# robustrobotics/multi_view_stereonet

Measured on AMD Instinct MI355X. Metric: depthmaps/sec at 512x256, 64 hypotheses, 2 src views; L1 vs ref, higher is better.
Workload: dtype f32; 1 GPU; GTA-SfM-shaped 512x256, D=64 hypotheses, 2 source views, cost-volume filter + 5 refiners; global_batch=256, parallelism=dp1 (independent images, all-gather of metric rows)

## Files before the change

### include/mvsn_hip.h

```cpp
#ifndef MVSN_HIP_H
#define MVSN_HIP_H

#include <stddef.h>
#include <stdint.h>

#ifdef __cplusplus
extern "C" {
#endif

#define MVSN_ABI_VERSION 6

#define MVSN_E_BADARG (-1)
#define MVSN_E_TOOLARGE (-2)
#define MVSN_E_WORKSPACE (-3)

typedef void *mvsn_stream_t;

int mvsn_abi_version(void);
const char *mvsn_last_error(void);

int mvsn_plane_sweep_setup(const float *T_right_in_left, const float *K_lvl0, const float *K_lvl4,
                           int n_chains, int rows4, int cols4, int num_idepth_samples,
                           float *idepth_samples, float *H_lvl4, float *H_inc, float *H_lvl0_plane0,
                           float *baseline, mvsn_stream_t stream);
// ... 132 lines not shown
                         uint8_t *out, mvsn_stream_t stream);
int mvsn_fusion_gather(const float *maps, const int *view, const int *pixel, int n_views, long pixels_per_view,
                       long count, float *out, mvsn_stream_t stream);

int mvsn_channel_l2_norm(const float *x, int n, int channels, long pixels, float *out, mvsn_stream_t stream);
int mvsn_idepth_scale(const float *prior, const float *fx, int n, long pixels, float *out, mvsn_stream_t stream);
int mvsn_refiner_epilogue(const float *prior, const float *fx, const float *delta, int n, long pixels, float *out,
                          mvsn_stream_t stream);

int mvsn_upsample_bilinear(const float *in, int n, int channels, int rows_in, int cols_in, int rows_out,
                           int cols_out, float *out, mvsn_stream_t stream);
int mvsn_upsample_prior(const float *in, const float *fx, int n, int rows_in, int cols_in, int rows_out, int cols_out,
                        float *out, float *out_scaled, mvsn_stream_t stream);
int mvsn_upsample_mask(const uint8_t *in, int n, int channels, int rows_in, int cols_in, int rows_out,
                       int cols_out, uint8_t *out, mvsn_stream_t stream);

int mvsn_area_downsample(const float *in, int n, int channels, int rows_in, int cols_in, float *out,
                         mvsn_stream_t stream);

int mvsn_image_pyramid_supported(int rows, int cols, int levels);
int mvsn_image_pyramid(const float *in, int n, int channels, int rows, int cols, int levels, float *const *out_levels,
                       mvsn_stream_t stream);
int mvsn_prepare_cameras(const float *K, const float *T_right_in_left, int batch, int n_sources, int levels,
                         const int *level_sizes_dev, float *K_pyr, float *T_normalised, float *T_inverse_normalised,
                         float *baseline, mvsn_stream_t stream);

int mvsn_fuse_sources(const float *raw, const float *refined, const float *baseline, const uint8_t *mask,
                      int n_sources, int batch, int num_idepth_samples, int pixels, int refined_aliases_raw,
                      float *raw_out, float *refined_out, uint8_t *mask_out, mvsn_stream_t stream);

// ... 73 lines not shown
                       int64_t *result, void *workspace, size_t workspace_bytes, mvsn_stream_t stream);
int mvsn_tsdf_extract(const float *sdf_sum, const float *weight, const float *color_sum, int nx, int ny, int nz,
                      float voxel_size, float origin_x, float origin_y, float origin_z, float min_weight,
                      const void *workspace, size_t workspace_bytes, long n_vertices, long n_quads, float *vertices,
                      float *normals, uint8_t *colors, int64_t *faces, int64_t *cell, mvsn_stream_t stream);

int mvsn_copy(void *dst, const void *src, size_t nbytes, mvsn_stream_t stream);
int mvsn_copy_many(void *const *dst, const void *const *src, const size_t *nbytes, int count, mvsn_stream_t stream);
int mvsn_gather_focal(const float *const *K_pyr, int levels, int batch, float *fx, mvsn_stream_t stream);
int mvsn_gather_strided(const float *src, int count, long stride, float *dst, mvsn_stream_t stream);

int mvsn_debug_set_band_flags(int flags);

int mvsn_debug_set_wino_rowphase(int mode);

int mvsn_debug_wino_plan(const mvsn_conv_desc *desc, int carrying, int out[8]);

int mvsn_debug_conv_plan(const mvsn_conv_desc *desc, int mode, int out[8]);

int mvsn_selftest_mfma(mvsn_stream_t stream);

#ifdef __cplusplus
}
#endif
#endif
```

### multi_view_stereonet_amd/_native.py

```python
import ctypes
import os
from ctypes import c_char_p, c_int, c_long, c_size_t, c_void_p, POINTER, Structure

import torch

_LIB_PATH = os.path.join(os.path.dirname(os.path.abspath(__file__)), "libmvsn_hip.so")
_lib = None


class ConvDesc(Structure):
    _fields_ = [("n", c_int), ("c_in", c_int), ("c_out", c_int), ("depth", c_int), ("rows", c_int),
                ("cols", c_int), ("kd", c_int), ("kh", c_int), ("kw", c_int), ("stride", c_int),
                ("dilation", c_int), ("precision", c_int)]


class ApplyJob(Structure):
    _fields_ = [("x", c_void_p), ("stats", c_void_p), ("gamma", c_void_p), ("beta", c_void_p),
                ("residual", c_void_p), ("r_stats", c_void_p), ("r_gamma", c_void_p), ("r_beta", c_void_p),
                ("out", c_void_p), ("n", c_int), ("reverse", c_int), ("spatial", c_long)]


class TowerDesc(Structure):
    _fields_ = [("inp", c_void_p * 3), ("channels", c_int * 3), ("sample_mod", c_int * 3), ("block_scale", c_void_p),
                ("scale_mod", c_int), ("scale_block", c_int), ("head_chunks", c_int), ("n_blocks", c_int),
# ... 35 lines not shown
    "mvsn_conv_winograd_supported": (c_int, [POINTER(ConvDesc)]),
    "mvsn_conv_packed_floats": (c_size_t, [POINTER(ConvDesc)]),
    "mvsn_conv_pack_weights": (c_int, [POINTER(ConvDesc), c_void_p, c_void_p, c_void_p]),
    "mvsn_conv_num_tiles": (c_int, [POINTER(ConvDesc)]),
    "mvsn_conv_forward": (c_int, [POINTER(ConvDesc)] + [c_void_p] * 10 + [c_void_p]),
    "mvsn_conv_forward_blocks": (c_int, [POINTER(ConvDesc), c_void_p, POINTER(c_int), c_int] + [c_void_p] * 4 + [c_void_p]),
    "mvsn_conv_forward_carry": (c_int, [POINTER(ConvDesc)] + [c_void_p] * 8 + [POINTER(ApplyJob), POINTER(c_int), c_void_p]),
    "mvsn_groupnorm_finalize": (c_int, [c_void_p, c_int, c_int, c_void_p, c_void_p]),
    "mvsn_groupnorm_finalize_split_workspace_bytes": (c_size_t, [c_int, c_int]),
    "mvsn_groupnorm_finalize_split": (c_int, [c_void_p, c_int, c_int, c_void_p, c_void_p, c_size_t, c_void_p]),
    "mvsn_groupnorm_lrelu_apply": (c_int, [c_void_p] * 5 + [c_int, c_long, c_void_p, c_void_p]),
    "mvsn_groupnorm_lrelu_add2": (c_int, [c_void_p] * 8 + [c_int, c_long, c_void_p, c_void_p]),
    "mvsn_conv_to1_block": (c_int, [c_void_p] * 9 + [c_int] * 3 + [c_void_p, c_void_p]),
    "mvsn_debug_set_band_flags": (c_int, [c_int]),
    "mvsn_debug_set_wino_rowphase": (c_int, [c_int]),
    "mvsn_debug_wino_plan": (c_int, [POINTER(ConvDesc), c_int, POINTER(c_int * 8)]),
    "mvsn_debug_conv_plan": (c_int, [POINTER(ConvDesc), c_int, POINTER(c_int * 8)]),
    "mvsn_copy_many": (c_int, [c_void_p, c_void_p, c_void_p, c_int, c_void_p]),
    "mvsn_conv_to1_block_records": (c_int, [c_void_p] * 2 + [c_int] + [c_void_p] * 7 + [c_int] * 3 + [c_void_p, c_void_p]),
    "mvsn_groupnorm_lrelu_apply_records": (c_int, [c_void_p] * 2 + [c_int] + [c_void_p] * 6 + [c_int, c_long, c_void_p, c_void_p]),
    "mvsn_conv_to1_supported": (c_int, [c_int, c_int]),
    "mvsn_conv_to1_volume_norm": (c_int, [c_void_p] * 6 + [c_int] * 4 + [c_void_p, c_void_p]),
    "mvsn_conv_to1": (c_int, [c_void_p] * 5 + [c_int] * 5 + [c_void_p, c_void_p]),
    "mvsn_soft_argmin": (c_int, [c_void_p] * 2 + [c_int] * 3 + [c_void_p, c_void_p]),
    "mvsn_soft_argmin_confidence": (c_int, [c_void_p] * 2 + [c_int] * 3 + [c_void_p] * 2 + [c_void_p]),
    "mvsn_confidence_fuse_sources": (c_int, [c_void_p] + [c_int] * 3 + [c_void_p, c_void_p]),
    "mvsn_confidence_mask": (c_int, [c_void_p, c_void_p, c_long, ctypes.c_float, c_void_p, c_void_p]),
    "mvsn_fusion_gather": (c_int, [c_void_p] * 3 + [c_int, c_long, c_long, c_void_p, c_void_p]),
    "mvsn_channel_l2_norm": (c_int, [c_void_p, c_int, c_int, c_long, c_void_p, c_void_p]),
    "mvsn_idepth_scale": (c_int, [c_void_p, c_void_p, c_int, c_long, c_void_p, c_void_p]),
    "mvsn_refiner_epilogue": (c_int, [c_void_p, c_void_p, c_void_p, c_int, c_long, c_void_p, c_void_p]),
    "mvsn_upsample_bilinear": (c_int, [c_void_p] + [c_int] * 6 + [c_void_p, c_void_p]),
    "mvsn_upsample_prior": (c_int, [c_void_p, c_void_p] + [c_int] * 5 + [c_void_p] * 3),
    "mvsn_upsample_mask": (c_int, [c_void_p] + [c_int] * 6 + [c_void_p, c_void_p]),
    "mvsn_image_pyramid_supported": (c_int, [c_int] * 3),
    "mvsn_image_pyramid": (c_int, [c_void_p] + [c_int] * 5 + [POINTER(c_void_p), c_void_p]),
    "mvsn_prepare_cameras": (c_int, [c_void_p] * 2 + [c_int] * 3 + [c_void_p] * 5 + [c_void_p]),
    "mvsn_area_downsample": (c_int, [c_void_p] + [c_int] * 4 + [c_void_p, c_void_p]),
    "mvsn_fuse_sources": (c_int, [c_void_p] * 4 + [c_int] * 5 + [c_void_p] * 3 + [c_void_p]),
    "mvsn_idepth_reproject_blocks": (c_int, [c_int]),
    "mvsn_idepth_reproject": (c_int, [c_void_p] * 5 + [c_int] * 3 + [c_void_p] * 6 + [c_void_p]),
    "mvsn_occlusion_mask": (c_int, [c_void_p] * 4 + [c_int] * 2 + [c_void_p, c_void_p]),
    "mvsn_masked_l1": (c_int, [c_void_p] * 4 + [c_long, c_int, c_void_p, c_void_p]),
    "mvsn_tower_16x32": (c_int, [POINTER(TowerDesc), c_int, c_void_p]),
    "mvsn_depth_metrics_blocks": (c_int, [c_long]),
    "mvsn_depth_metrics": (c_int, [c_void_p] * 3 + [c_int, c_long, ctypes.c_float, ctypes.c_float, c_void_p, c_void_p, c_void_p]),
    "mvsn_fusion_workspace_bytes": (c_size_t, [c_int] * 4),
    "mvsn_fusion_consistency": (c_int, [c_void_p] * 6 + [c_int] * 5 + [ctypes.c_float] * 2 + [c_int] + [c_void_p] * 4 +
                                [c_size_t, c_void_p]),
# ... 132 lines not shown
```

### multi_view_stereonet_amd/csrc/mvsn_conv_wino.hip

```cpp
#include <type_traits>
#include <utility>

#include "mvsn_resident.h"
#include "mvsn_conv_wino.h"

namespace mvsn {

constexpr int WN_THREADS = 512, WN_WAVES = 8;
constexpr int WN_TY = 16, WN_TX = 32;
constexpr int WN_WIDE_TY = 10, WN_WIDE_TX = 40, WN_WIDE_PC = WN_WIDE_TX / 2, WN_WIDE_NP = (WN_WIDE_TY / 2) * WN_WIDE_PC;
constexpr int WN_ROLL_PR = 6, WN_ROLL_NP = WN_ROLL_PR * WN_WIDE_PC, WN_ROLL_HY = 2 * WN_ROLL_PR + 3;
constexpr int WN_TILE_RP = 3;
constexpr int wn_pa(int dil) { return (dil + 3) / 4 * 4; }
constexpr int WN_UFLOATS = 16 * 128;
constexpr int WN_MAX_CHUNKS = 9;
constexpr int WN_LDS_MAX = 160 * 1024;

__device__ floatx4 g_wn_zero16 = {0.f, 0.f, 0.f, 0.f};

#ifndef MVSN_WN_ABLATE
#define MVSN_WN_ABLATE 0
#endif

#ifndef MVSN_RD_ABLATE
// ... 167 lines not shown
  return WinoDiv{(unsigned)m, s};
}
__device__ __forceinline__ int wdiv(int n, WinoDiv f) { return (int)((__umulhi((unsigned)n, f.mul) + (unsigned)n) >> f.shift); }

struct WinoArgs {
  int n, cin, H, W, ntx, tiles, nchunks;
  WinoDiv fd_ntx;
  int cb0, cb1;
  const float *in1, *in2;
  size_t bs0, cs0;
  int rev;
  int D;
  int pr;
  WinoDiv fd_pr;
  int nty, rpy;
};

struct RideArgs {
  const float *x, *stats, *gamma, *beta;
  const float *res, *r_stats, *r_gamma, *r_beta;
  float *out;
  int units;
  WinoDiv fd_upp;
};
typedef const __attribute__((address_space(4))) float *wn_cfloat;
__device__ __forceinline__ float wn_sload(const float *p, size_t i) { return ((wn_cfloat)(size_t)p)[i]; }

__global__ void wino_pack_kernel(const float *__restrict__ w, int cin, int cout, int nchunks, int kd,
                                 float *__restrict__ out) {
  const int total = nchunks * WN_UFLOATS;
// ... 64 lines not shown
  const int nsteps = (g.nchunks + KS - 1) / KS;
  const int uchunks = VOL ? NSTAGE * KS : nsteps * KS;

  const int tid = threadIdx.x, lane = tid & 63;
  const int wave = __builtin_amdgcn_readfirstlane(tid >> 6);
  const size_t plane = (size_t)g.H * g.W;
  const int ptiles = ROLL ? g.tiles : (RP ? DIL * g.rpy * g.ntx : g.D * g.tiles);
  auto roll_item = [&](int t, int &zA, int &prA0, int &sA) {
    const int R0 = t * WN_ROLL_PR;
    zA = wdiv(R0, g.fd_pr);
    prA0 = R0 - zA * g.pr;
    sA = g.pr - prA0 < WN_ROLL_PR ? g.pr - prA0 : WN_ROLL_PR;
  };
  const int total = g.n * ptiles;
  const int G = gridDim.x;
  const int slot = xcd_tile_index(blockIdx.x, G);
#ifdef MVSN_WN_STAMPS
  unsigned long long *dbg = (blockIdx.x == gridDim.x / 3 && tid == 0) ? g_wn_stamps : nullptr;
  unsigned long long *dbg_lds = reinterpret_cast<unsigned long long *>(U + L.stamps(uchunks));
  int dbg_i = 0;
  bool dbg_on = true;
#endif
  WN_STAMP();

  if constexpr (!VOL) {
    const int runs = g.nchunks * (WN_UFLOATS / 256);
    for (int run = wave; run < runs; run += WN_WAVES)
      wn_dma16<ASM_DMA>(upk + (size_t)run * 256 + lane * 4, U + run * 256);
    if (uchunks != g.nchunks)
      *reinterpret_cast<floatx4 *>(U + g.nchunks * WN_UFLOATS + tid * 4) = floatx4{0.f, 0.f, 0.f, 0.f};
// ... 2 lines not shown
  float *bias_lds = U + L.bias(uchunks);
  if (tid < 32) bias_lds[tid] = bias ? bias[tid] : 0.0f;

  constexpr int STEP_PIECES = KS * 4 * PIECES;
  constexpr bool EVEN = STEP_PIECES % WN_WAVES == 0;
  constexpr int PER = EVEN ? STEP_PIECES / WN_WAVES : 2;
  static_assert(EVEN || (KS == 1 && PIECES == 3), "uneven DMA split only for the 12-piece case");
  static_assert(!EVEN || PIECES % PER == 0 || PER % PIECES == 0, "a wave's pieces stay within one channel");
  const int dch = EVEN ? (wave * PER) / PIECES : (wave & 3);
  const int dp0 = EVEN ? (wave * PER) % PIECES : (wave < 4 ? 0 : 2);
  const int dpn = EVEN ? (PER < PIECES ? PER : PIECES) : (wave < 4 ? 2 : 1);
  const float *zero = reinterpret_cast<const float *>(&g_wn_zero16);
  int pf_round = 0, pf_chunk = 0, pf_stage = 0;
  int pf_goff[PER];
  int pf_n = 0, pf_z = 0;
  bool pf_live = slot < total;
  int rd_young = 0;
  auto pf_plan = [&]() {
    const int flat = g.rev ? total - 1 - (pf_round * G + slot) : pf_round * G + slot;
    const int n = flat / ptiles;
    int tile = flat - n * ptiles;
    int r_pr0 = 0, r_s = WN_ROLL_PR;
    if constexpr (ROLL) {
      roll_item(tile, pf_z, r_pr0, r_s);
      tile = 0;
    } else if constexpr (VOL) {
      pf_z = tile / g.tiles;
      tile -= pf_z * g.tiles;
    }
    const int tyi = ROLL ? 0 : wdiv(tile, g.fd_ntx), txi = tile - tyi * g.ntx;
    const int y0 = ROLL ? 2 * r_pr0 : item_y0(tyi), x0 = txi * TX;
    pf_n = n;
    int lo;
    asm volatile("v_mbcnt_lo_u32_b32 %0, -1, 0\n\tv_mbcnt_hi_u32_b32 %0, -1, %0" : "=v"(lo));
#pragma unroll
    for (int i = 0; i < PER; ++i) {
      const int e = (dp0 + i) * 64 + lo;
      const int row = e / DQ, q = e - row * DQ;
      int gy = y0 - DIL + YS * row;
      const int gx = x0 - PA + 4 * q;
      int zsh = 0;
      if constexpr (ROLL) {
        const bool isb = (r_s < WN_ROLL_PR) & (row >= 2 * r_s + 1);
        gy = isb ? row - (2 * r_s + 2) : gy;
        zsh = isb ? g.H * g.W : 0;
      }
      const bool ok = (i < dpn) & (e < GROUPS) & (gy >= 0) & (gy < g.H) & (gx >= 0) & (gx < g.W);
      pf_goff[i] = ok ? (zsh + gy * g.W + gx) * (MVSN_WN_BUFDMA ? 4 : 1) : -1;
    }
  };
  auto pf_issue = [&]() {
    if (!pf_live) return;
    rd_young += PER;
    bool cok;
    const float *src;
    unsigned rbytes = 0;
    bool roll_first = false;
    if constexpr (ROLL) {
      const int kz = pf_chunk >> 2, c = (pf_chunk & 3) * 8 + dch, zz = pf_z + kz - 1;
      cok = zz >= 0 && zz < g.D;
      roll_first = zz < 0;
      const int zlo = zz < 0 ? 0 : zz, zhi = zz + 1 < g.D ? zz + 1 : g.D - 1;
      const int np = zhi - zlo + 1 > 0 ? zhi - zlo + 1 : 0;
      const int zsel = zlo < g.D - 1 ? zlo : g.D - 1;
      src = in + (size_t)(unsigned)__builtin_amdgcn_readfirstlane((pf_n * 32 + c) * g.D + zsel) * plane;
      rbytes = (unsigned)np * (unsigned)plane * 4u;
// ... 19 lines not shown
          if constexpr (ROLL) {
            static_assert(!ROLL || MVSN_WN_BUFDMA, "rolling strips: descriptor DMA only");
            unsigned off = (unsigned)pf_goff[i];
            off -= roll_first ? (unsigned)plane * 4u : 0u;
            wn_dma16_buf<ASM_DMA>(src, pbytes, off, dst + (dp0 + i) * 256);
          } else if constexpr (MVSN_WN_BUFDMA) {
            wn_dma16_buf<ASM_DMA>(src, pbytes, (unsigned)pf_goff[i], dst + (dp0 + i) * 256);
          } else {
            const float *p = (cok && pf_goff[i] >= 0) ? src + pf_goff[i] : zero;
            wn_dma16<ASM_DMA>(p, dst + (dp0 + i) * 256);
          }
        }
      }
    }
    pf_stage = pf_stage + 1 == NSTAGE ? 0 : pf_stage + 1;
    if (++pf_chunk == nsteps) {
      pf_chunk = 0;
      ++pf_round;
      pf_live = pf_round * G + slot < total;
      if (pf_live) pf_plan();
    }
  };
  int uq_chunk = 0, uq_stage = 0, uq_left = 0;
  auto uq_issue = [&]() {
    if constexpr (VOL) {
      if (uq_left <= 0) return;
      --uq_left;
      rd_young += 2;
      const float *src = upk + (size_t)uq_chunk * UST + wave * 512 + lane * 4;
      float *dst = U + uq_stage * UST + wave * 512;
      wn_dma16<ASM_DMA>(src, dst);
      wn_dma16<ASM_DMA>(src + 256, dst + 256);
      uq_stage = uq_stage + 1 == NSTAGE ? 0 : uq_stage + 1;
      uq_chunk = uq_chunk + 1 == nsteps ? 0 : uq_chunk + 1;
    }
  };
  if (pf_live) pf_plan();
  if constexpr (VOL) uq_left = slot < total ? ((total - slot + G - 1) / G) * nsteps : 0;
#pragma unroll
  for (int i = 0; i < NSTAGE; ++i) {
    pf_issue();
    if (i < NSTAGE - 1) uq_issue();
  }
  WN_STAMP();

  const int pcol = lane & 15, kc = lane >> 4;
  int ya = RP ? 2 * wave : (wave / DIL) * 2 * DIL + wave % DIL, xa = (pcol / DIL) * 2 * DIL + pcol % DIL;
  int lane_pr = 0;
  if constexpr (WIDE != 0) {
    const int q = wave * 16 + pcol, qq = q < NP ? q : 0;
    const int pr = qq / WN_WIDE_PC;
    lane_pr = pr;
    ya = 2 * pr, xa = 2 * (qq - pr * WN_WIDE_PC);
  }
  const int my_items = slot < total ? (total - slot + G - 1) / G : 0;
  const int total_steps = my_items * nsteps;

  constexpr int PERV = PER + (VOL ? 2 : 0);
  static_assert(!VOL || EVEN, "volume form: every wave issues the same number of pieces");
  static_assert(RIDE == 0 || EVEN, "carried jobs: layers with an even DMA split");
  auto wait_landed = [&](int younger) {
#define WN_WAIT_CASE(K)                                                              \
  case K:                                                                            \
    if (EVEN) asm volatile("s_waitcnt vmcnt(%0)" ::"n"(PERV * (K)) : "memory");        \
    else if (wave < 4) asm volatile("s_waitcnt vmcnt(%0)" ::"n"(2 * (K)) : "memory"); \
    else asm volatile("s_waitcnt vmcnt(%0)" ::"n"(K) : "memory");                       \
    break;
    switch (younger) {
      WN_WAIT_CASE(0)
      WN_WAIT_CASE(1)
      WN_WAIT_CASE(2)
      WN_WAIT_CASE(3)
      WN_WAIT_CASE(4)
      default:
        WN_WAIT_CASE(5)
    }
#undef WN_WAIT_CASE
  };
  static_assert(NSTAGE - 1 <= 5 && PERV * 5 <= 63, "wait_landed covers up to 5 younger steps within the vmcnt range");

  int xf_round = 0, xf_chunk = 0, xf_stage = 0;
  unsigned xf_mask = 0;
  unsigned xf_maska = 0, xf_maskb = 0;
  float xf_sc = 0.f, xf_sh = 0.f;
  bool xf_on = false;
  auto xf_prepare = [&]() {
    if constexpr (MODE == 1) {
      const int lin = xf_round * G + slot;
      const int flat = g.rev ? total - 1 - lin : lin;
      xf_on = lin < total;
      if (!xf_on) return;
      const int n = flat / ptiles;
      int tile = flat - n * ptiles, z = 0;
      int r_pr0 = 0, r_s = WN_ROLL_PR;
      if constexpr (ROLL) {
        roll_item(tile, z, r_pr0, r_s);
        tile = 0;
      } else if constexpr (VOL) {
        z = tile / g.tiles;
        tile -= z * g.tiles;
      }
      if (xf_chunk == 0) {
        const int tyi = ROLL ? 0 : wdiv(tile, g.fd_ntx), txi = tile - tyi * g.ntx;
        const int y0 = ROLL ? 2 * r_pr0 : item_y0(tyi), x0 = txi * TX;
        xf_mask = 0;
        xf_maska = xf_maskb = 0;
        int lo;
        asm volatile("v_mbcnt_lo_u32_b32 %0, -1, 0\n\tv_mbcnt_hi_u32_b32 %0, -1, %0" : "=v"(lo));
#pragma unroll
        for (int i = 0; i < PER; ++i) {
          const int e = (dp0 + i) * 64 + lo;
          const int row = e / DQ, q = e - row * DQ;
          int gy = y0 - DIL + YS * row;
          const int gx = x0 - PA + 4 * q;
          bool isb = false;
          if constexpr (ROLL) {
            isb = r_s < WN_ROLL_PR && row >= 2 * r_s + 1;
            if (isb) gy = row - (2 * r_s + 2);
          }
          if (i < dpn && e < GROUPS && gy >= 0 && gy < g.H && gx >= 0 && gx < g.W) {
            if constexpr (ROLL) (isb ? xf_maskb : xf_maska) |= 1u << i;
            else xf_mask |= 1u << i;
          }
        }
      }
      int c = xf_chunk * (KS * 4) + dch;
      bool live = c < g.cin;
      if constexpr (VOL) {
        const int zz = z + (xf_chunk >> 2) - 1;
        c = (xf_chunk & 3) * 8 + dch;
        live = zz >= 0 && zz < g.D;
        if constexpr (ROLL) {
          const bool liveb = zz + 1 < g.D;
          xf_mask = (live ? xf_maska : 0u) | (liveb ? xf_maskb : 0u);
          live = live || liveb;
        }
      }
      if (live) {
        const float mean = in_stats[((size_t)n * 4 + (c >> 3)) * 2 + 0];
        const float rstd = in_stats[((size_t)n * 4 + (c >> 3)) * 2 + 1];
        xf_sc = rstd * in_gamma[c];
        xf_sh = in_beta[c] - mean * xf_sc;
      } else {
        xf_on = false;
      }
// ... 9 lines not shown
            float *q = dst + (dp0 + i) * 256;
            if constexpr (SHIFT || CSHIFT % 4 != 0) {
              float e[4] = {q[0], q[1], q[2], q[3]};
#pragma unroll
              for (int r = 0; r < 4; ++r) e[r] = lrelu02(e[r] * xf_sc + xf_sh);
              q[0] = e[0], q[1] = e[1], q[2] = e[2], q[3] = e[3];
            } else {
              floatx4 v = *reinterpret_cast<floatx4 *>(q);
#pragma unroll
              for (int r = 0; r < 4; ++r) v[r] = lrelu02(v[r] * xf_sc + xf_sh);
              *reinterpret_cast<floatx4 *>(q) = v;
            }
          }
      }
      xf_stage = xf_stage + 1 == NSTAGE ? 0 : xf_stage + 1;
      if (++xf_chunk == nsteps) xf_chunk = 0, ++xf_round;
    }
  };

  int tr_round = 0, tr_chunk = 0, tr_stage = 0;
  auto tr_setup = [&]() {
    if constexpr (ROLL) {
      const int lin = tr_round * G + slot;
      if (lin < total) {
        const int flat = g.rev ? total - 1 - lin : lin;
        int zA, prA0, sA;
        roll_item(flat - (flat / ptiles) * ptiles, zA, prA0, sA);
        ya = 2 * lane_pr + (lane_pr >= sA ? 1 : 0);
      }
    }
  };
// ... 347 lines not shown
#pragma unroll
      for (int t = 0; t < 2; ++t) qv[t] = sum16(qv[t]);
      if (pc < 4) {
        float *rec = out_partials + (((size_t)n * ptiles + (ROLL ? (size_t)0 : (size_t)z * g.tiles) + tile_id) * WN_WAVES + wave) * 48;
        rec += gq * 12 + pc * 3;
        const int ga = gq >> 1;
        const bool a = pc == ga, b = pc == 2 + ga;
        rec[0] = (a || b) ? npos : 0.f;
        rec[1] = a ? m[0] : (b ? m[1] : 0.f);
        rec[2] = a ? qv[0] : (b ? qv[1] : 0.f);
      }
    }
  };

  int step = 0, mm_stage = 0;
  for (int round = 0; round < my_items; ++round) {
#ifdef MVSN_WN_STAMPS
    dbg_on = round >= 3 || my_items < 4;
#endif
    const int flat = g.rev ? total - 1 - (round * G + slot) : round * G + slot;
    const int n = flat / ptiles;
    int tile_id = flat - n * ptiles, z = 0;
    int r_pr0 = 0, r_s = WN_ROLL_PR;
    if constexpr (ROLL) {
      roll_item(tile_id, z, r_pr0, r_s);
    } else if constexpr (VOL) {
      z = tile_id / g.tiles;
      tile_id -= z * g.tiles;
    }
    const int tyi = ROLL ? 0 : wdiv(tile_id, g.fd_ntx), txi = ROLL ? 0 : tile_id - tyi * g.ntx;
    const int y0 = ROLL ? 2 * r_pr0 : item_y0(tyi), x0 = txi * TX;

#pragma unroll
    for (int xi = 0; xi < 16; ++xi) asm volatile("" : "=v"(acc[xi][0]), "=v"(acc[xi][1]));

    int chunk = 0;
    auto do_step = [&](auto firstc) {
      const bool has_next = step + 1 < total_steps;
      bool waited = false;
      if constexpr (RIDE > 0) {
        if (rd_young == PERV) asm volatile("s_waitcnt vmcnt(%0)" ::"n"(PERV) : "memory");
        else if (rd_young == PER) asm volatile("s_waitcnt vmcnt(%0)" ::"n"(PER) : "memory");
        else if (VOL && rd_young == 2) asm volatile("s_waitcnt vmcnt(2)" ::: "memory");
        else asm volatile("s_waitcnt vmcnt(0)" ::: "memory");
        rd_consume(lane);
        waited = true;
      }
      if (has_next) {
        const int rest = total_steps - (step + 2);
        if (!waited) wait_landed(rest < 0 ? 0 : (rest < NSTAGE - 2 ? rest : NSTAGE - 2));
        xf_apply();
// ... 34 lines not shown
          if (xi + 1 < 16 && !(MVSN_WN_ABLATE & 2)) {
            fb[cur ^ 1][0] = ub[(xi + 1) * 128];
            fb[cur ^ 1][1] = ub[(xi + 1) * 128 + 64];
          }
          if constexpr (FIRST) {
            acc[xi][0] = TR ? mfma16x16x4(fb[cur][0], v[h][xi], floatx4{0.f, 0.f, 0.f, 0.f})
                            : mfma16x16x4(v[h][xi], fb[cur][0], floatx4{0.f, 0.f, 0.f, 0.f});
            acc[xi][1] = TR ? mfma16x16x4(fb[cur][1], v[h][xi], floatx4{0.f, 0.f, 0.f, 0.f})
                            : mfma16x16x4(v[h][xi], fb[cur][1], floatx4{0.f, 0.f, 0.f, 0.f});
          } else {
            acc[xi][0] = TR ? mfma16x16x4(fb[cur][0], v[h][xi], acc[xi][0]) : mfma16x16x4(v[h][xi], fb[cur][0], acc[xi][0]);
            acc[xi][1] = TR ? mfma16x16x4(fb[cur][1], v[h][xi], acc[xi][1]) : mfma16x16x4(v[h][xi], fb[cur][1], acc[xi][1]);
          }
          if (h == 0 && xi == 1 && has_next && !(MVSN_WN_ABLATE & 4)) {
            pf_issue();
            uq_issue();
          }
          if constexpr (INTER) {
            if (!(MVSN_WN_ABLATE & 1)) {
              v[h][xi] = tj == 0 ? tc[0] - tc[2] : (tj == 1 ? tc[1] + tc[2] : (tj == 2 ? tc[2] - tc[1] : tc[1] - tc[3]));
              if (MVSN_WN_PIN) asm volatile("" : "+v"(v[h][xi]));
            }
            if (tj == 3) {
#pragma unroll
              for (int k = 0; k < 4; ++k) tc[k] = tn[k];
            }
          }
          __builtin_amdgcn_sched_barrier(0);
        }
        if constexpr (!INTER) {
          if (!(MVSN_WN_ABLATE & 1)) {
            tr_finish(dn, v, h, h + 1);
#pragma unroll
            for (int xi = 0; xi < 16; ++xi)
              if (MVSN_WN_PIN) asm volatile("" : "+v"(v[h][xi]));
          }
          __builtin_amdgcn_sched_barrier(0);
        }
      };
      multiply(firstc, std::integral_constant<int, 0>{});
      if constexpr (KS == 2) multiply(std::false_type{}, std::integral_constant<int, 1>{});
      tr_advance();
      if constexpr (VOL) mm_stage = mm_stage + 1 == NSTAGE ? 0 : mm_stage + 1;
      WN_STAMP();
      ++step;
    };
    do_step(std::true_type{});
    for (chunk = 1; chunk < nsteps; ++chunk) do_step(std::false_type{});
    if (!(MVSN_WN_ABLATE & 16) || n < 0) {
      if constexpr (TR) finish_tile_tr(n, z, tile_id, y0, x0, r_s);
      else finish_tile(n, z, tile_id, y0, x0);
    }
  }
  if constexpr (RIDE > 0) {
    if (total_steps > 0) {
      asm volatile("s_waitcnt vmcnt(0)" ::: "memory");
      int ln;
      asm volatile("v_mbcnt_lo_u32_b32 %0, -1, 0\n\tv_mbcnt_hi_u32_b32 %0, -1, %0" : "=v"(ln));
      rd_consume(ln);
    }
  }
#ifdef MVSN_WN_STAMPS
  if (dbg)
// ... 193 lines not shown
        for (int a = 0; a < 2; ++a) {
          const bool rok = y0 + a < g.Ho;
          const unsigned so = rok ? (unsigned)((tt * 16 * oplane + (y0 + a) * g.Wo + x0) * 4) : 0u;
          wn_store4<0>(osrd, rok ? ovoff[0] : 0xFFFFFFFFu, so, floatx4{y[0][a][0], y[0][a][1], y[1][a][0], y[1][a][1]});
          wn_store4<0>(osrd, rok ? ovoff[1] : 0xFFFFFFFFu, so, floatx4{y[2][a][0], y[2][a][1], y[3][a][0], y[3][a][1]});
        }
      }
#pragma unroll
      for (int xi = 0; xi < 16; ++xi) acc[xi][0] = acc[xi][1] = floatx4{0.f, 0.f, 0.f, 0.f};
      ++item;
    }
  }
}

static int g_wn_rowphase = 0;

bool wino_geom(const mvsn_conv_desc *d, WinoGeom *g) {
  if (!d || d->precision != MVSN_CONV_FP32_WINO) return false;
  g->rpy = 0;
  if (d->n <= 0 || d->c_in <= 0 || d->c_out != 32 || d->depth < 1 || d->rows <= 0 || d->cols <= 0) return false;
  g->s2 = false;
  if (d->kd == 1 && d->kh == 5 && d->kw == 5 && d->stride == 2) {
    if (d->c_in != 32 || d->dilation != 1 || d->depth != 1 || d->cols % 8 != 0) return false;
    if ((unsigned long long)d->rows * d->cols * 32ull * 4ull >= (1ull << 31)) return false;
    g->s2 = true, g->wide = 0;
    g->n = d->n, g->cin = 32, g->H = d->rows, g->W = d->cols, g->dil = 1, g->D = 1, g->vol = false;
    g->nty = ((d->rows - 1) / 2 + 1 + S2_TY - 1) / S2_TY;
    g->ntx = ((d->cols - 1) / 2 + 1 + S2_TX - 1) / S2_TX;
    g->tiles = g->nty * g->ntx;
    g->nchunks = S2_STEPS * 4;
// ... 121 lines not shown
      return MVSN_E_BADARG;
    }
    rd.x = job->x, rd.stats = job->stats, rd.gamma = job->gamma, rd.beta = job->beta;
    rd.res = job->residual, rd.r_stats = job->r_stats, rd.r_gamma = job->r_gamma, rd.r_beta = job->r_beta;
    rd.out = job->out;
    rd.units = (int)((long)job->n * 32 * (job->spatial / 256));
    rd.fd_upp = wino_div((unsigned)(job->spatial / 256));
  }
  WinoArgs a;
  a.n = g.n, a.cin = g.cin, a.H = g.H, a.W = g.W, a.ntx = g.ntx, a.tiles = g.tiles, a.nchunks = g.nchunks;
  a.fd_ntx = wino_div((unsigned)g.ntx);
  a.cb0 = g.cin, a.cb1 = 0, a.in1 = a.in2 = in;
  a.D = g.D;
  a.pr = (g.H + 1) / 2, a.fd_pr = wino_div((unsigned)a.pr);
  a.nty = g.nty, a.rpy = g.rpy;
  if (blocks) a.cb0 = blocks->cb0, a.cb1 = blocks->cb1, a.in1 = blocks->in1, a.in2 = blocks->in2;
  a.rev = (job && job->reverse == 1) ? 1 : 0;
  a.cs0 = (size_t)g.H * g.W, a.bs0 = (size_t)a.cb0 * a.cs0;
  if (blocks && blocks->cs0) a.cs0 = blocks->cs0, a.bs0 = blocks->bs0;
  const int row = wino_select(g, job != nullptr);
  if (row < 0) {
    set_error("mvsn_conv_forward(winograd): no kernel form for this layer");
    return MVSN_E_BADARG;
  }
  const size_t lds = WN_FORMS[row].bytes(g.nchunks);
  const int cus = device_cus();
  const long total = (long)g.n * wino_work_items(g);
  const dim3 grid((unsigned)(total < cus ? total : cus));
  auto launch = [&](auto mode, auto I) -> int {
    constexpr WinoForm F = WN_FORMS[decltype(I)::value];
// ... 10 lines not shown
  if (int rc = with_form_row(row, std::make_index_sequence<WN_NFORMS>{}, [&](auto I) {
        return xf ? launch(std::integral_constant<int, 1>{}, I) : launch(std::integral_constant<int, 0>{}, I);
      }))
    return rc;
  return check_launch("mvsn_conv_forward(winograd)");
}

}

extern "C" int mvsn_debug_set_wino_rowphase(int mode) {
  const int old = mvsn::g_wn_rowphase;
  mvsn::g_wn_rowphase = mode;
  return old;
}

extern "C" int mvsn_debug_wino_plan(const mvsn_conv_desc *desc, int carrying, int out[8]) {
  mvsn::WinoGeom g;
  if (!out || !mvsn::wino_geom(desc, &g)) return 0;
  const int row = mvsn::wino_select(g, carrying != 0);
  if (row < 0) return 0;
  const mvsn::WinoForm &f = mvsn::WN_FORMS[row];
  out[0] = f.ks, out[1] = f.nstage, out[2] = f.ride, out[3] = f.tile, out[4] = f.fullw;
  out[5] = (int)f.bytes(g.nchunks), out[6] = (int)mvsn::wino_work_items(g), out[7] = f.nsteps(g.nchunks);
  return 1;
}

#ifdef MVSN_WN_STAMPS
extern "C" int mvsn_debug_set_wino_stamps(void *buf) {
  return (int)hipMemcpyToSymbol(HIP_SYMBOL(mvsn::g_wn_stamps), &buf, sizeof(buf));
}
// ... 2 lines not shown
```

### multi_view_stereonet_amd/csrc/mvsn_misc.hip

```cpp
#include <type_traits>

#include "mvsn_geom.h"
#include "mvsn_resident.h"

namespace mvsn {

__global__ __launch_bounds__(256) void soft_argmin_kernel(const float *__restrict__ cost,
                                                          const float *__restrict__ samples, int D, int P,
                                                          float *__restrict__ out) {
  const int p = blockIdx.x * blockDim.x + threadIdx.x;
  const int n = blockIdx.y;
  if (p >= P) return;
  const float *c = cost + (size_t)n * D * P + p;
  const float *s = samples + (size_t)n * D;
  float m = -INFINITY;
  int d0 = 0;
  for (; d0 + 16 <= D; d0 += 16) {
    float v[16];
#pragma unroll
    for (int j = 0; j < 16; ++j) v[j] = c[(size_t)(d0 + j) * P];
#pragma unroll
    for (int j = 0; j < 16; ++j) m = fmaxf(m, -v[j]);
  }
  for (int d = d0; d < D; ++d) m = fmaxf(m, -c[(size_t)d * P]);
// ... 136 lines not shown
                                                              uint8_t *__restrict__ out) {
  const size_t gid = (size_t)blockIdx.x * blockDim.x + threadIdx.x;
  if (gid >= total_groups) return;
  const int gx = (int)(gid % groups_per_row);
  const size_t rowid = gid / groups_per_row;
  const uint2 w = *reinterpret_cast<const uint2 *>(in + rowid * win + gx * 8);
  typedef unsigned u32x4 __attribute__((ext_vector_type(4)));
  u32x4 o;
  o[0] = __builtin_amdgcn_perm(w.x, w.x, 0x01010000u);
  o[1] = __builtin_amdgcn_perm(w.x, w.x, 0x03030202u);
  o[2] = __builtin_amdgcn_perm(w.y, w.y, 0x01010000u);
  o[3] = __builtin_amdgcn_perm(w.y, w.y, 0x03030202u);
  uint8_t *dst = out + (rowid * 2) * (size_t)(win * 2) + gx * 16;
  __builtin_nontemporal_store(o, reinterpret_cast<u32x4 *>(dst));
  __builtin_nontemporal_store(o, reinterpret_cast<u32x4 *>(dst + win * 2));
}

__global__ __launch_bounds__(256) void area_downsample_kernel(const float *__restrict__ in, int hin, int win,
                                                              int hout, int wout, float *__restrict__ out) {
  const int x = blockIdx.x * blockDim.x + threadIdx.x;
  const int y = blockIdx.y;
  const size_t plane = blockIdx.z;
  if (x >= wout) return;
  const int y0 = (y * hin) / hout, y1 = ((y + 1) * hin + hout - 1) / hout;
  const int x0 = (x * win) / wout, x1 = ((x + 1) * win + wout - 1) / wout;
  const float *ip = in + plane * hin * win;
  float sum = 0.0f;
  for (int yy = y0; yy < y1; ++yy)
    for (int xx = x0; xx < x1; ++xx) sum += ip[yy * win + xx];
  out[(plane * hout + y) * wout + x] = sum / (float)((y1 - y0) * (x1 - x0));
// ... 202 lines not shown
  MVSN_REQUIRE(in && out, MVSN_E_BADARG, "mvsn_upsample_mask: null pointer");
  MVSN_REQUIRE(n > 0 && channels > 0 && rows_in > 0 && cols_in > 0 && rows_out > 0 && cols_out > 0, MVSN_E_BADARG,
               "mvsn_upsample_mask: bad sizes");
  const int groups_per_row = (cols_out + 15) / 16;
  const size_t total = (size_t)n * channels * rows_out * groups_per_row;
  MVSN_REQUIRE((total + 255) / 256 < 2147483647ull, MVSN_E_TOOLARGE, "mvsn_upsample_mask: grid");
  if (rows_out == 2 * rows_in && cols_out == 2 * cols_in && cols_in % 8 == 0 && (((size_t)in | (size_t)out) & 15) == 0) {
    const size_t groups = (size_t)n * channels * rows_in * (cols_in / 8);
    hipLaunchKernelGGL(mvsn::upsample_mask2x_kernel, dim3((unsigned)((groups + 255) / 256)), dim3(256), 0,
                       (hipStream_t)stream, in, rows_in, cols_in, cols_in / 8, groups, out);
    return mvsn::check_launch("mvsn_upsample_mask(2x)");
  }
  hipLaunchKernelGGL(mvsn::upsample_mask16_kernel, dim3((unsigned)((total + 255) / 256)), dim3(256), 0,
                     (hipStream_t)stream, in, rows_in, cols_in, rows_out, cols_out, groups_per_row, total, out);
  return mvsn::check_launch("mvsn_upsample_mask");
}

extern "C" int mvsn_area_downsample(const float *in, int n, int channels, int rows_in, int cols_in, float *out,
                                    mvsn_stream_t stream) {
  MVSN_REQUIRE(in && out, MVSN_E_BADARG, "mvsn_area_downsample: null pointer");
  MVSN_REQUIRE(n > 0 && channels > 0 && rows_in > 0 && cols_in > 0, MVSN_E_BADARG, "mvsn_area_downsample: bad sizes");
  const int rows_out = (rows_in + 1) / 2, cols_out = (cols_in + 1) / 2;
  MVSN_REQUIRE((long)n * channels <= 65535 && rows_out <= 65535, MVSN_E_TOOLARGE, "mvsn_area_downsample: grid");
  dim3 grid((cols_out + 255) / 256, rows_out, n * channels);
  hipLaunchKernelGGL(mvsn::area_downsample_kernel, grid, dim3(256), 0, (hipStream_t)stream, in, rows_in, cols_in,
                     rows_out, cols_out, out);
  return mvsn::check_launch("mvsn_area_downsample");
}

extern "C" int mvsn_fuse_sources(const float *raw, const float *refined, const float *baseline, const uint8_t *mask,
// ... 536 lines not shown
```

### multi_view_stereonet_amd/multi_view_stereonet.py

```python
import ctypes
import threading
import warnings
from typing import Dict, List, Optional

import torch
import torch.nn as nn

from . import _native
from .params import REFINER_DILATIONS, build_parameter_tree

ListTensor = List[torch.Tensor]


class _Conv:

    def __init__(self, lib, weight: torch.Tensor, bias: Optional[torch.Tensor], stride: int = 1, dilation: int = 1):
        self.lib = lib
        self.cout, self.cin = int(weight.shape[0]), int(weight.shape[1])
        self.dims = weight.dim() - 2
        k = tuple(int(s) for s in weight.shape[2:])
        self.kd, self.kh, self.kw = (k if self.dims == 3 else (1,) + k)
        self.stride, self.dilation = stride, dilation
        self.bias = bias.detach().contiguous().float() if bias is not None else None
        self.weight = weight.detach().contiguous().float() if self.cout == 1 else None
# ... 955 lines not shown
        assert c == 1
        out = self.empty((n, 1, int(size[0]), int(size[1])), dtype=torch.float32, device=x.device)
        scaled = self.empty(out.shape, out.dtype, out.device)
        self._call("mvsn_upsample_prior", self.lib.mvsn_upsample_prior, _native.ptr(x), _native.ptr(fx), n, h, w,
                   int(size[0]), int(size[1]), _native.ptr(out), _native.ptr(scaled), _native.stream(),
                   nbytes=4.0 * (x.numel() + 2 * out.numel()))
        return out, scaled

    def upsample_mask(self, m: torch.Tensor, size) -> torch.Tensor:
        n, c, h, w = m.shape
        out = self.empty((n, c, int(size[0]), int(size[1])), dtype=torch.bool, device=m.device)
        self._call("mvsn_upsample_mask", self.lib.mvsn_upsample_mask, _native.ptr(m), n, c, h, w, int(size[0]),
                   int(size[1]), _native.ptr(out), _native.stream(), nbytes=float(m.numel() + out.numel()))
        return out

    def fuse_sources(self, raw, refined, baseline, mask, S, B, alias):
        N, D, rows, cols = mask.shape
        dev = raw.device
        raw_out = self.empty((B, 1, rows, cols), dtype=torch.float32, device=dev)
        ref_out = self.empty((B, 1, rows, cols), dtype=torch.float32, device=dev)
        mask_out = self.empty((B, D, rows, cols), dtype=torch.bool, device=dev)
        self._call("mvsn_fuse_sources", self.lib.mvsn_fuse_sources, _native.ptr(raw), _native.ptr(refined),
                   _native.ptr(baseline), _native.ptr(mask), S, B, D, rows * cols, 1 if alias else 0,
                   _native.ptr(raw_out), _native.ptr(ref_out), _native.ptr(mask_out), _native.stream(),
                   nbytes=float(mask.numel() + mask_out.numel()))
        return raw_out, ref_out, mask_out

    def forward(self, left_image_pyr, K_pyr, T_right_in_lefts, right_image_pyrs, D, do_filter, do_refiners,
                capture: Optional[dict] = None):
        S = len(T_right_in_lefts)
# ... 48 lines not shown
        if capture is not None:
            capture.update(idepth_samples=samples, H=H4, H_inc=Hinc, H_lvl0_plane0=H0, baseline=baseline,
                           warped_fullres=warped0, left_features=left_feats, plane0_features=plane0,
                           cost_volume=cost, mask_volume=mask, feature_volume=fvol, filtered_cost=filtered,
                           raw_per_chain=raw)
            if want_conf:
                capture.update(confidence_per_chain=conf_chain)

        idepth = [None] * 5
        prior = [None] * 5
        masks = [None] * 5
        prior[4], idepth[4], masks[4] = raw4, idepth4, mask4
        conf = [None] * 5
        if want_conf:
            conf[4] = self.confidence_fuse_sources(conf_chain, S, B)
        for lvl in (3, 2, 1, 0):
            size = left_image_pyr[lvl].shape[-2:]
            if want_conf:
                conf[lvl] = self.upsample(conf[lvl + 1], size)
            if do_refiners[lvl]:
                fx = fx_all[lvl]
                prior[lvl], scaled = self.upsample_prior(idepth[lvl + 1], fx, size)
            else:
                prior[lvl] = self.upsample(idepth[lvl + 1], size)
            masks[lvl] = self.upsample_mask(masks[lvl + 1], size)
            if do_refiners[lvl]:
                img = self.f32c(left_image_pyr[lvl])
                guide = [img] if lvl == 0 else [img, left_feats[lvl]]
                idepth[lvl] = self.idepth_refiner(lvl, guide, prior[lvl], fx, scaled=scaled)
            else:
                idepth[lvl] = prior[lvl]
        out = {"left_idepthmap_pyr": idepth, "left_idepthmap_raw_pyr": prior, "left_idepthmap_mask_pyr": masks}
        if want_conf:
            out["left_confidence_pyr"] = conf
        return out


class MultiViewStereoNet(nn.Module):

    num_levels = 5
# ... 212 lines not shown
```

Measured before the change: 3856 depthmaps/s.

## Skip zero-padded depth taps in Winograd volume conv and fuse mask pyramid upsampling

```diff
diff --git a/include/mvsn_hip.h b/include/mvsn_hip.h
--- a/include/mvsn_hip.h
+++ b/include/mvsn_hip.h
@@ -170,6 +170,8 @@
                         float *out, float *out_scaled, mvsn_stream_t stream);
 int mvsn_upsample_mask(const uint8_t *in, int n, int channels, int rows_in, int cols_in, int rows_out,
                        int cols_out, uint8_t *out, mvsn_stream_t stream);
+int mvsn_upsample_mask_pyramid(const uint8_t *in, int n, int channels, int rows_in, int cols_in, int levels,
+                               uint8_t *out1, uint8_t *out2, uint8_t *out3, uint8_t *out4, mvsn_stream_t stream);
 
 int mvsn_area_downsample(const float *in, int n, int channels, int rows_in, int cols_in, float *out,
                          mvsn_stream_t stream);
@@ -273,6 +275,8 @@
 
 int mvsn_debug_set_wino_rowphase(int mode);
 
+int mvsn_debug_set_wino_zero_taps(int on);
+
 int mvsn_debug_wino_plan(const mvsn_conv_desc *desc, int carrying, int out[8]);
 
 int mvsn_debug_conv_plan(const mvsn_conv_desc *desc, int mode, int out[8]);
diff --git a/multi_view_stereonet_amd/_native.py b/multi_view_stereonet_amd/_native.py
--- a/multi_view_stereonet_amd/_native.py
+++ b/multi_view_stereonet_amd/_native.py
@@ -73,6 +73,7 @@
     "mvsn_conv_to1_block": (c_int, [c_void_p] * 9 + [c_int] * 3 + [c_void_p, c_void_p]),
     "mvsn_debug_set_band_flags": (c_int, [c_int]),
     "mvsn_debug_set_wino_rowphase": (c_int, [c_int]),
+    "mvsn_debug_set_wino_zero_taps": (c_int, [c_int]),
     "mvsn_debug_wino_plan": (c_int, [POINTER(ConvDesc), c_int, POINTER(c_int * 8)]),
     "mvsn_debug_conv_plan": (c_int, [POINTER(ConvDesc), c_int, POINTER(c_int * 8)]),
     "mvsn_copy_many": (c_int, [c_void_p, c_void_p, c_void_p, c_int, c_void_p]),
@@ -92,6 +93,7 @@
     "mvsn_upsample_bilinear": (c_int, [c_void_p] + [c_int] * 6 + [c_void_p, c_void_p]),
     "mvsn_upsample_prior": (c_int, [c_void_p, c_void_p] + [c_int] * 5 + [c_void_p] * 3),
     "mvsn_upsample_mask": (c_int, [c_void_p] + [c_int] * 6 + [c_void_p, c_void_p]),
+    "mvsn_upsample_mask_pyramid": (c_int, [c_void_p] + [c_int] * 5 + [c_void_p] * 4 + [c_void_p]),
     "mvsn_image_pyramid_supported": (c_int, [c_int] * 3),
     "mvsn_image_pyramid": (c_int, [c_void_p] + [c_int] * 5 + [POINTER(c_void_p), c_void_p]),
     "mvsn_prepare_cameras": (c_int, [c_void_p] * 2 + [c_int] * 3 + [c_void_p] * 5 + [c_void_p]),
diff --git a/multi_view_stereonet_amd/csrc/mvsn_conv_wino.hip b/multi_view_stereonet_amd/csrc/mvsn_conv_wino.hip
--- a/multi_view_stereonet_amd/csrc/mvsn_conv_wino.hip
+++ b/multi_view_stereonet_amd/csrc/mvsn_conv_wino.hip
@@ -205,6 +205,7 @@
   int pr;
   WinoDiv fd_pr;
   int nty, rpy;
+  int ztaps;
 };
 
 struct RideArgs {
@@ -299,6 +300,12 @@
   };
   const int total = g.n * ptiles;
   const int G = gridDim.x;
+  constexpr bool ZT = VOL && RIDE == 0 && WIDE != 2;
+  auto zt_first = [&](int z) { return (g.ztaps && z == 0) ? 4 : 0; };
+  auto zt_end = [&](int z) { return (g.ztaps && z == g.D - 1) ? 8 : 12; };
+  auto zt_first_r = [&](int r) { return (g.ztaps && r < g.tiles) ? 4 : 0; };
+  auto zt_end_r = [&](int r) { return (g.ztaps && r >= ptiles - g.tiles) ? 8 : 12; };
+  auto rev_walk = [&]() { return ZT ? 0 : g.rev; };
   const int slot = xcd_tile_index(blockIdx.x, G);
 #ifdef MVSN_WN_STAMPS
   unsigned long long *dbg = (blockIdx.x == gridDim.x / 3 && tid == 0) ? g_wn_stamps : nullptr;
@@ -331,10 +338,11 @@
   int pf_round = 0, pf_chunk = 0, pf_stage = 0;
   int pf_goff[PER];
   int pf_n = 0, pf_z = 0;
+  unsigned pf_hist = 0xFFFFu;
   bool pf_live = slot < total;
   int rd_young = 0;
   auto pf_plan = [&]() {
-    const int flat = g.rev ? total - 1 - (pf_round * G + slot) : pf_round * G + slot;
+    const int flat = rev_walk() ? total - 1 - (pf_round * G + slot) : pf_round * G + slot;
     const int n = flat / ptiles;
     int tile = flat - n * ptiles;
     int r_pr0 = 0, r_s = WN_ROLL_PR;
@@ -344,6 +352,7 @@
     } else if constexpr (VOL) {
       pf_z = tile / g.tiles;
       tile -= pf_z * g.tiles;
+      if constexpr (ZT) pf_chunk = zt_first(pf_z);
     }
     const int tyi = ROLL ? 0 : wdiv(tile, g.fd_ntx), txi = tile - tyi * g.ntx;
     const int y0 = ROLL ? 2 * r_pr0 : item_y0(tyi), x0 = txi * TX;
@@ -367,6 +376,7 @@
     }
   };
   auto pf_issue = [&]() {
+    if constexpr (ZT) pf_hist = (pf_hist << 8) | (pf_live ? (unsigned)pf_chunk : 255u);
     if (!pf_live) return;
     rd_young += PER;
     bool cok;
@@ -416,7 +426,10 @@
       }
     }
     pf_stage = pf_stage + 1 == NSTAGE ? 0 : pf_stage + 1;
-    if (++pf_chunk == nsteps) {
+    bool pf_wrap;
+    if constexpr (ZT) pf_wrap = ++pf_chunk == zt_end(pf_z);
+    else pf_wrap = ++pf_chunk == nsteps;
+    if (pf_wrap) {
       pf_chunk = 0;
       ++pf_round;
       pf_live = pf_round * G + slot < total;
@@ -424,25 +437,39 @@
     }
   };
   int uq_chunk = 0, uq_stage = 0, uq_left = 0;
-  auto uq_issue = [&]() {
-    if constexpr (VOL) {
+  auto uq_issue = [&](int behind) {
+    if constexpr (ZT) {
+      uq_chunk = (int)((pf_hist >> (behind ? 8 : 0)) & 255u);
+      if (uq_chunk == 255) return;
+    } else if constexpr (VOL) {
       if (uq_left <= 0) return;
       --uq_left;
+    }
+    if constexpr (VOL) {
       rd_young += 2;
       const float *src = upk + (size_t)uq_chunk * UST + wave * 512 + lane * 4;
       float *dst = U + uq_stage * UST + wave * 512;
       wn_dma16<ASM_DMA>(src, dst);
       wn_dma16<ASM_DMA>(src + 256, dst + 256);
       uq_stage = uq_stage + 1 == NSTAGE ? 0 : uq_stage + 1;
-      uq_chunk = uq_chunk + 1 == nsteps ? 0 : uq_chunk + 1;
+      if constexpr (!ZT) uq_chunk = uq_chunk + 1 == nsteps ? 0 : uq_chunk + 1;
     }
   };
   if (pf_live) pf_plan();
-  if constexpr (VOL) uq_left = slot < total ? ((total - slot + G - 1) / G) * nsteps : 0;
+  int zt_steps = 0;
+  if constexpr (ZT) {
+    const int rstep = G % ptiles;
+    for (int lin = slot, r = slot % ptiles; lin < total; lin += G) {
+      zt_steps += zt_end_r(r) - zt_first_r(r);
+      r = r + rstep >= ptiles ? r + rstep - ptiles : r + rstep;
+    }
+  } else if constexpr (VOL) {
+    uq_left = slot < total ? ((total - slot + G - 1) / G) * nsteps : 0;
+  }
 #pragma unroll
   for (int i = 0; i < NSTAGE; ++i) {
     pf_issue();
-    if (i < NSTAGE - 1) uq_issue();
+    if (i < NSTAGE - 1) uq_issue(0);
   }
   WN_STAMP();
 
@@ -456,7 +483,8 @@
     ya = 2 * pr, xa = 2 * (qq - pr * WN_WIDE_PC);
   }
   const int my_items = slot < total ? (total - slot + G - 1) / G : 0;
-  const int total_steps = my_items * nsteps;
+  int total_steps = my_items * nsteps;
+  if constexpr (ZT) total_steps = zt_steps;
 
   constexpr int PERV = PER + (VOL ? 2 : 0);
   static_assert(!VOL || EVEN, "volume form: every wave issues the same number of pieces");
@@ -481,7 +509,7 @@
   };
   static_assert(NSTAGE - 1 <= 5 && PERV * 5 <= 63, "wait_landed covers up to 5 younger steps within the vmcnt range");
 
-  int xf_round = 0, xf_chunk = 0, xf_stage = 0;
+  int xf_round = 0, xf_chunk = ZT ? -1 : 0, xf_stage = 0;
   unsigned xf_mask = 0;
   unsigned xf_maska = 0, xf_maskb = 0;
   float xf_sc = 0.f, xf_sh = 0.f;
@@ -489,7 +517,7 @@
   auto xf_prepare = [&]() {
     if constexpr (MODE == 1) {
       const int lin = xf_round * G + slot;
-      const int flat = g.rev ? total - 1 - lin : lin;
+      const int flat = rev_walk() ? total - 1 - lin : lin;
       xf_on = lin < total;
       if (!xf_on) return;
       const int n = flat / ptiles;
@@ -502,7 +530,15 @@
         z = tile / g.tiles;
         tile -= z * g.tiles;
       }
-      if (xf_chunk == 0) {
+      bool xf_new = false;
+      int xf_c = xf_chunk;
+      if constexpr (ZT) {
+        const int late = 12 - zt_end(z);
+        xf_new = xf_chunk < 0;
+        if (xf_new) xf_chunk = zt_first(z) + late;
+        xf_c = xf_chunk - late;
+      }
+      if (ZT ? xf_new : xf_chunk == 0) {
         const int tyi = ROLL ? 0 : wdiv(tile, g.fd_ntx), txi = tile - tyi * g.ntx;
         const int y0 = ROLL ? 2 * r_pr0 : item_y0(tyi), x0 = txi * TX;
         xf_mask = 0;
@@ -526,11 +562,11 @@
           }
         }
       }
-      int c = xf_chunk * (KS * 4) + dch;
+      int c = xf_c * (KS * 4) + dch;
       bool live = c < g.cin;
       if constexpr (VOL) {
-        const int zz = z + (xf_chunk >> 2) - 1;
-        c = (xf_chunk & 3) * 8 + dch;
+        const int zz = z + (xf_c >> 2) - 1;
+        c = (xf_c & 3) * 8 + dch;
         live = zz >= 0 && zz < g.D;
         if constexpr (ROLL) {
           const bool liveb = zz + 1 < g.D;
@@ -570,7 +606,7 @@
           }
       }
       xf_stage = xf_stage + 1 == NSTAGE ? 0 : xf_stage + 1;
-      if (++xf_chunk == nsteps) xf_chunk = 0, ++xf_round;
+      if (++xf_chunk == (ZT ? 12 : nsteps)) xf_chunk = ZT ? -1 : 0, ++xf_round;
     }
   };
 
@@ -948,11 +984,11 @@
   };
 
   int step = 0, mm_stage = 0;
-  for (int round = 0; round < my_items; ++round) {
+  for (int round = 0; ZT ? round * G + slot < total : round < my_items; ++round) {
 #ifdef MVSN_WN_STAMPS
     dbg_on = round >= 3 || my_items < 4;
 #endif
-    const int flat = g.rev ? total - 1 - (round * G + slot) : round * G + slot;
+    const int flat = rev_walk() ? total - 1 - (round * G + slot) : round * G + slot;
     const int n = flat / ptiles;
     int tile_id = flat - n * ptiles, z = 0;
     int r_pr0 = 0, r_s = WN_ROLL_PR;
@@ -969,6 +1005,7 @@
     for (int xi = 0; xi < 16; ++xi) asm volatile("" : "=v"(acc[xi][0]), "=v"(acc[xi][1]));
 
     int chunk = 0;
+    if constexpr (ZT) chunk = zt_first(z);
     auto do_step = [&](auto firstc) {
       const bool has_next = step + 1 < total_steps;
       bool waited = false;
@@ -1033,7 +1070,7 @@
           }
           if (h == 0 && xi == 1 && has_next && !(MVSN_WN_ABLATE & 4)) {
             pf_issue();
-            uq_issue();
+            uq_issue(1);
           }
           if constexpr (INTER) {
             if (!(MVSN_WN_ABLATE & 1)) {
@@ -1062,10 +1099,15 @@
       tr_advance();
       if constexpr (VOL) mm_stage = mm_stage + 1 == NSTAGE ? 0 : mm_stage + 1;
       WN_STAMP();
-      ++step;
+      if constexpr (ZT) --total_steps;
+      else ++step;
     };
     do_step(std::true_type{});
-    for (chunk = 1; chunk < nsteps; ++chunk) do_step(std::false_type{});
+    if constexpr (ZT) {
+      for (const int end = zt_end(z); ++chunk < end;) do_step(std::false_type{});
+    } else {
+      for (chunk = 1; chunk < nsteps; ++chunk) do_step(std::false_type{});
+    }
     if (!(MVSN_WN_ABLATE & 16) || n < 0) {
       if constexpr (TR) finish_tile_tr(n, z, tile_id, y0, x0, r_s);
       else finish_tile(n, z, tile_id, y0, x0);
@@ -1289,6 +1331,7 @@
 }
 
 static int g_wn_rowphase = 0;
+static int g_wn_zero_taps = 1;
 
 bool wino_geom(const mvsn_conv_desc *d, WinoGeom *g) {
   if (!d || d->precision != MVSN_CONV_FP32_WINO) return false;
@@ -1440,6 +1483,7 @@
   a.D = g.D;
   a.pr = (g.H + 1) / 2, a.fd_pr = wino_div((unsigned)a.pr);
   a.nty = g.nty, a.rpy = g.rpy;
+  a.ztaps = g_wn_zero_taps ? 1 : 0;
   if (blocks) a.cb0 = blocks->cb0, a.cb1 = blocks->cb1, a.in1 = blocks->in1, a.in2 = blocks->in2;
   a.rev = (job && job->reverse == 1) ? 1 : 0;
   a.cs0 = (size_t)g.H * g.W, a.bs0 = (size_t)a.cb0 * a.cs0;
@@ -1480,6 +1524,12 @@
   return old;
 }
 
+extern "C" int mvsn_debug_set_wino_zero_taps(int on) {
+  const int old = mvsn::g_wn_zero_taps;
+  mvsn::g_wn_zero_taps = on ? 1 : 0;
+  return old;
+}
+
 extern "C" int mvsn_debug_wino_plan(const mvsn_conv_desc *desc, int carrying, int out[8]) {
   mvsn::WinoGeom g;
   if (!out || !mvsn::wino_geom(desc, &g)) return 0;
diff --git a/multi_view_stereonet_amd/csrc/mvsn_misc.hip b/multi_view_stereonet_amd/csrc/mvsn_misc.hip
--- a/multi_view_stereonet_amd/csrc/mvsn_misc.hip
+++ b/multi_view_stereonet_amd/csrc/mvsn_misc.hip
@@ -174,6 +174,64 @@
   uint8_t *dst = out + (rowid * 2) * (size_t)(win * 2) + gx * 16;
   __builtin_nontemporal_store(o, reinterpret_cast<u32x4 *>(dst));
   __builtin_nontemporal_store(o, reinterpret_cast<u32x4 *>(dst + win * 2));
+}
+
+constexpr int MP_ROWS = 16;
+template <int K>
+__device__ __forceinline__ void mask_pyramid_level(const uint8_t *__restrict__ src, int rows, int win, bool fast,
+                                                   uint8_t *__restrict__ dst) {
+  constexpr int F = 1 << K, NB = 16 / F;
+  typedef unsigned u32x4 __attribute__((ext_vector_type(4)));
+  const int wout = win * F;
+  if (fast) {
+    const int gpr = wout / 16, groups = rows * F * gpr;
+    for (int i = threadIdx.x; i < groups; i += blockDim.x) {
+      const int r = i / gpr, gx = i - r * gpr;
+      const uint8_t *p = src + (r >> K) * win + gx * NB;
+      u32x4 o;
+      if constexpr (K == 1) {
+        const uint2 w = *reinterpret_cast<const uint2 *>(p);
+        o[0] = __builtin_amdgcn_perm(w.x, w.x, 0x01010000u);
+        o[1] = __builtin_amdgcn_perm(w.x, w.x, 0x03030202u);
+        o[2] = __builtin_amdgcn_perm(w.y, w.y, 0x01010000u);
+        o[3] = __builtin_amdgcn_perm(w.y, w.y, 0x03030202u);
+      } else if constexpr (K == 2) {
+        const unsigned w = *reinterpret_cast<const unsigned *>(p);
+        o[0] = __builtin_amdgcn_perm(w, w, 0x00000000u);
+        o[1] = __builtin_amdgcn_perm(w, w, 0x01010101u);
+        o[2] = __builtin_amdgcn_perm(w, w, 0x02020202u);
+        o[3] = __builtin_amdgcn_perm(w, w, 0x03030303u);
+      } else if constexpr (K == 3) {
+        o[0] = o[1] = (unsigned)p[0] * 0x01010101u;
+        o[2] = o[3] = (unsigned)p[1] * 0x01010101u;
+      } else {
+        o[0] = o[1] = o[2] = o[3] = (unsigned)p[0] * 0x01010101u;
+      }
+      __builtin_nontemporal_store(o, reinterpret_cast<u32x4 *>(dst + (size_t)i * 16));
+    }
+  } else {
+    const int total = rows * F * wout;
+    for (int i = threadIdx.x; i < total; i += blockDim.x) {
+      const int r = i / wout, x = i - r * wout;
+      dst[i] = src[(r >> K) * win + (x >> K)];
+    }
+  }
+}
+
+__global__ __launch_bounds__(256) void upsample_mask_pyramid_kernel(const uint8_t *__restrict__ in, int hin, int win,
+                                                                    int levels, int fast, uint8_t *__restrict__ out1,
+                                                                    uint8_t *__restrict__ out2,
+                                                                    uint8_t *__restrict__ out3,
+                                                                    uint8_t *__restrict__ out4) {
+  const size_t plane = blockIdx.x;
+  const int y0 = blockIdx.y * MP_ROWS;
+  const int rows = hin - y0 < MP_ROWS ? hin - y0 : MP_ROWS;
+  const size_t at = (plane * hin + y0) * (size_t)win;
+  const uint8_t *src = in + at;
+  mask_pyramid_level<1>(src, rows, win, fast != 0, out1 + at * 4);
+  if (levels > 1) mask_pyramid_level<2>(src, rows, win, fast != 0, out2 + at * 16);
+  if (levels > 2) mask_pyramid_level<3>(src, rows, win, fast != 0, out3 + at * 64);
+  if (levels > 3) mask_pyramid_level<4>(src, rows, win, fast != 0, out4 + at * 256);
 }
 
 __global__ __launch_bounds__(256) void area_downsample_kernel(const float *__restrict__ in, int hin, int win,
@@ -406,6 +464,24 @@
   hipLaunchKernelGGL(mvsn::upsample_mask16_kernel, dim3((unsigned)((total + 255) / 256)), dim3(256), 0,
                      (hipStream_t)stream, in, rows_in, cols_in, rows_out, cols_out, groups_per_row, total, out);
   return mvsn::check_launch("mvsn_upsample_mask");
+}
+
+extern "C" int mvsn_upsample_mask_pyramid(const uint8_t *in, int n, int channels, int rows_in, int cols_in, int levels,
+                                          uint8_t *out1, uint8_t *out2, uint8_t *out3, uint8_t *out4,
+                                          mvsn_stream_t stream) {
+  MVSN_REQUIRE(levels >= 1 && levels <= 4, MVSN_E_BADARG, "mvsn_upsample_mask_pyramid: 1 to 4 levels");
+  uint8_t *const outs[4] = {out1, out2, out3, out4};
+  bool ptrs = in != nullptr, aligned = ((size_t)in & 15) == 0;
+  for (int k = 0; k < levels; ++k) ptrs = ptrs && outs[k] != nullptr, aligned = aligned && ((size_t)outs[k] & 15) == 0;
+  MVSN_REQUIRE(ptrs, MVSN_E_BADARG, "mvsn_upsample_mask_pyramid: null pointer");
+  MVSN_REQUIRE(n > 0 && channels > 0 && rows_in > 0 && cols_in > 0, MVSN_E_BADARG, "mvsn_upsample_mask_pyramid: bad sizes");
+  const unsigned long long planes = (unsigned long long)n * channels, ychunks = (rows_in + mvsn::MP_ROWS - 1) / mvsn::MP_ROWS;
+  MVSN_REQUIRE(planes < 2147483647ull && ychunks <= 65535 && (unsigned long long)cols_in * 256 * mvsn::MP_ROWS < (1ull << 31),
+               MVSN_E_TOOLARGE, "mvsn_upsample_mask_pyramid: grid");
+  const int fast = aligned && cols_in % 8 == 0;
+  hipLaunchKernelGGL(mvsn::upsample_mask_pyramid_kernel, dim3((unsigned)planes, (unsigned)ychunks), dim3(256), 0,
+                     (hipStream_t)stream, in, rows_in, cols_in, levels, fast, out1, out2, out3, out4);
+  return mvsn::check_launch("mvsn_upsample_mask_pyramid");
 }
 
 extern "C" int mvsn_area_downsample(const float *in, int n, int channels, int rows_in, int cols_in, float *out,
diff --git a/multi_view_stereonet_amd/multi_view_stereonet.py b/multi_view_stereonet_amd/multi_view_stereonet.py
--- a/multi_view_stereonet_amd/multi_view_stereonet.py
+++ b/multi_view_stereonet_amd/multi_view_stereonet.py
@@ -993,6 +993,17 @@
                    int(size[1]), _native.ptr(out), _native.stream(), nbytes=float(m.numel() + out.numel()))
         return out
 
+    def upsample_mask_pyramid(self, m: torch.Tensor, sizes):
+        n, c, h, w = m.shape
+        sizes = [(int(s[0]), int(s[1])) for s in sizes]
+        if not 1 <= len(sizes) <= 4 or any(s != (h << (k + 1), w << (k + 1)) for k, s in enumerate(sizes)):
+            return None
+        outs = [self.empty((n, c) + s, dtype=torch.bool, device=m.device) for s in sizes]
+        ptrs = [_native.ptr(o) for o in outs] + [None] * (4 - len(outs))
+        self._call("mvsn_upsample_mask_pyramid", self.lib.mvsn_upsample_mask_pyramid, _native.ptr(m), n, c, h, w,
+                   len(outs), *ptrs, _native.stream(), nbytes=float(m.numel() + sum(o.numel() for o in outs)))
+        return outs
+
     def fuse_sources(self, raw, refined, baseline, mask, S, B, alias):
         N, D, rows, cols = mask.shape
         dev = raw.device
@@ -1071,6 +1082,7 @@
         conf = [None] * 5
         if want_conf:
             conf[4] = self.confidence_fuse_sources(conf_chain, S, B)
+        mask_pyr = self.upsample_mask_pyramid(mask4, [left_image_pyr[lvl].shape[-2:] for lvl in (3, 2, 1, 0)])
         for lvl in (3, 2, 1, 0):
             size = left_image_pyr[lvl].shape[-2:]
             if want_conf:
@@ -1080,7 +1092,7 @@
                 prior[lvl], scaled = self.upsample_prior(idepth[lvl + 1], fx, size)
             else:
                 prior[lvl] = self.upsample(idepth[lvl + 1], size)
-            masks[lvl] = self.upsample_mask(masks[lvl + 1], size)
+            masks[lvl] = mask_pyr[3 - lvl] if mask_pyr is not None else self.upsample_mask(masks[lvl + 1], size)
             if do_refiners[lvl]:
                 img = self.f32c(left_image_pyr[lvl])
                 guide = [img] if lvl == 0 else [img, left_feats[lvl]]
```

New measurement: 3835 depthmaps/s. Within noise of the previous version (-0.6%).
